# danieleschmidt/spin-torque-rl-gym

Measured on AMD Instinct MI355X. Metric: env_steps_per_sec, higher is better.
Workload: dtype f64

## Files before the change

### spin-torque-rl-gym_amd/csrc/stg_kernels.hpp

```cpp
#pragma once
#include "../../include/spintorque_hip.h"
#include "stg_launch_plan.hpp"
#include "stg_physics.hpp"

#include <hip/hip_runtime.h>

#include <type_traits>

using namespace stg;

struct alignas(16) EnvRec {
    double m[3];
    double tgt[3];
    double etot;
    uint32_t stepw;
    uint32_t rng;
};
static_assert(sizeof(EnvRec) == 64, "state record size");
constexpr uint32_t STG_DONE_BIT = 0x80000000u;

struct StateView {
    EnvRec* rec;
};

// ... 368 lines not shown
            const V3 ref{row[C_REFX], row[C_REFY], row[C_REFZ]};
            const double r = resistance(m, (int)row[C_DEVTYPE], row[C_RP], row[C_RAP], row[C_TMR], ref, row[C_RSERIES]);
            const double v = J * r * row[C_AREA];
            energy = (v * v) / r * T;
        }
        if (so.ok) {
            const double inv = rsqrt_fast(dot(so.m, so.m));
            m = V3{so.m.x * inv, so.m.y * inv, so.m.z * inv};
        }
        etot += energy;
        step += 1;
        rng += 1;
        const double align = dot(m, tgt);
        is_success = align >= a.c.thr;
        reward = 10.0 * (is_success ? 10.0 : 0.0);
        reward += (-a.c.w_energy) * (-energy / 1e-12);
        reward += (align - prev_align);
        if (isnan(reward) || isinf(reward)) reward = -1.0;
        reward = fmin(fmax(reward, -1e6), 1e6);
        truncated = step >= a.c.max_steps;
        st = so.ok ? (so.resets > 0 ? STG_STATUS_RESET : STG_STATUS_OK) : STG_STATUS_NOOP;
        c_steps += 1; c_sub += (unsigned long long)so.work; c_noop += so.ok ? 0 : 1;
        done = is_success || truncated;
    }
    const bool do_reset = a.autoreset && done && live;
    if (wr && do_reset && a.final_obs) {
        if (a.records) {
            float o[12];
            make_obs(o, m, tgt, row, a.c, step, etot, J, T);
            float2* fo = (float2*)(a.final_obs + (ko * N + i) * 12);
#pragma unroll
            for (int q = 0; q < 6; ++q) fo[q] = make_float2(o[2 * q], o[2 * q + 1]);
        } else {
            write_obs(a.final_obs + ko * 12 * N, N, i, m, tgt, row, a.c, step, etot, J, T);
        }
    }
    if (do_reset) {
        device_reset_draw(a.c.seed, env_id, rng, a.c, true, true, m, tgt);
        etot = 0.0; step = 0; done = false;
        J = 0.0; T = 0.0;
    }
    if (wr) {
        if (a.records) {
            write_record((char*)a.obs + ko * N * STG_RECORD_BYTES, i, m, tgt, row, a.c, step, etot, J, T, (float)reward,
                         (is_success ? 1u : 0u) | (truncated ? 0x100u : 0u) | ((uint32_t)st << 16));
        } else {
            write_obs(a.obs + ko * 12 * N, N, i, m, tgt, row, a.c, step, etot, J, T);
            a.reward[ko * N + i] = (float)reward;
            a.term[ko * N + i] = is_success ? 1 : 0;
            a.trunc[ko * N + i] = truncated ? 1 : 0;
        }
        if (a.reward64) a.reward64[ko * N + i] = reward;
        if (a.energy) a.energy[ko * N + i] = energy;
        if (a.status) a.status[ko * N + i] = st;
    }
}

constexpr int REFILL_STRIPES = 64;
constexpr int REFILL_CURSOR_STRIDE = 16;

template <bool THERMAL, bool MULTI, bool AXIS_Z, typename AT, bool IDS>
__device__ __forceinline__ void refill_wave(const StepArgs& a, int64_t w, int64_t nw, int64_t blk0, int64_t nblk_q, int lane, const double* s_tab,
                                            unsigned long long& c_steps, unsigned long long& c_sub, unsigned long long& c_noop) {
    const int64_t N = a.N;
    const int64_t tiles = (N + TILE_ENVS - 1) / TILE_ENVS;
    if (w == 0 && lane < REFILL_STRIPES) a.refill_cursor_next[lane * REFILL_CURSOR_STRIDE] = 0ull;
    const AT* act = (const AT*)a.actions;
    const Recorder norec{};
    const LlgsEnergyK noek{};
    const Dp5Tab tb = make_dp5_tab();
    InlineNormals ns;

    int64_t i = 0, o = 0;
    bool has_env = false;
    double J = 0.0, T = 0.0;
    V3 e_tgt{0.0, 0.0, 1.0};
    double e_etot = 0.0;
    int32_t e_step = 0;
    uint32_t e_rng = 0;
    bool e_skip = false;
    const double* row = a.ctab;
    LlgsK k = load_llgs(row);
    LlgsLane L;
    L.active = false; L.idle = true; L.rejected = false; L.attempts = 0; L.npts = 0;
    L.y = L.f = L.m0 = V3{0.0, 0.0, 1.0};
    L.t = L.T = L.h_abs = L.min_step = L.bJ = L.bpJ = 0.0;
    V3 out_m{0.0, 0.0, 1.0};

    auto take = [&](int64_t p, bool want) {
        const int64_t idx = blk0 + (p >> 6);
        const bool valid_blk = want && (p >> 6) < nblk_q;
        const int64_t slot = (valid_blk ? refill_slot_base(idx, tiles) : 0) + (p & 63);
        const bool valid = valid_blk && slot < N;
        if (!valid) return;
        if constexpr (IDS) {
            o = a.perm ? (int64_t)a.perm[slot] : slot;
            const uint32_t id = a.ids[o];
            if ((int64_t)id >= a.n_state) { write_bad_id(a, o); return; }
            i = (int64_t)id;
        } else {
            i = a.perm ? (int64_t)a.perm[slot] : slot;
        }
        V3 m;
        bool done;
        load_state(a.s, i, m, e_tgt, e_etot, e_step, e_rng, done);
        const uint32_t rng = e_rng;
        if (a.perm) {
            typedef typename std::conditional<std::is_same<AT, double>::value, double2, float2>::type AT2;
            const AT2 aa = ((const AT2*)a.act_sorted)[slot];
            parse_action<AT>(aa.x, aa.y, a.c.max_current, a.c.max_duration, J, T);
        } else {
            const int64_t p = IDS ? o : i;
            parse_action<AT>(act[p], act[N + p], a.c.max_current, a.c.max_duration, J, T);
        }
        if (MULTI) {
            const int c = (int)a.cls[i];
            row = s_tab + (c < a.ncls ? c : 0) * C_COUNT;
            k = load_llgs(row);
        }
        const RngKey rk{a.c.seed, (uint64_t)(a.env_id0 + i), rng};
        e_skip = a.c.skip_done && done;
        llgs_lane_begin<THERMAL, false, AXIS_Z>(L, out_m, m, J, T, k, row[C_BETA], row[C_BETAP], a.c.rtol, a.c.atol, a.c.max_step, rk,
                                                norec, noek, ns, !e_skip);
        has_env = true;
    };
    auto finish = [&]() {
        const SolveOut so = llgs_lane_finish<false>(L, out_m, norec, noek, ns);
        V3 m = L.m0, tgt = e_tgt;
        double etot = e_etot;
        int32_t step = e_step;
        uint32_t rng = e_rng;
        bool done = e_skip;
        env_step_tail(a, IDS ? o : i, 0, true, true, !e_skip, row, (uint64_t)(a.env_id0 + i), m, tgt, etot, step, rng, done, J, T, so, c_steps, c_sub, c_noop);
        store_state(a.s, i, m, tgt, etot, step, rng, done);
        has_env = false;
        L.active = false;
    };

    take(w * 64 + lane, true);
    const int64_t n_rest = nblk_q > nw ? nblk_q - nw : 0;
    static_assert(REFILL_STRIPES == 64, "one lane per stripe when a wavefront looks for a stripe that still has entries");
    int stripe = (int)(w % REFILL_STRIPES);
    bool queue_open = true;
    int64_t loc_q = 0, loc_end = 0;
    int loc_stripe = 0, full_streak = 0;
    bool more = n_rest > 0;
    const int check = a.refill_check > 0 ? a.refill_check : 1;
    for (;;) {
        LlgsMasks M = llgs_masks_open(L);
        for (int c = 0; c < check; ++c) {
            llgs_lane_gate<false>(L, M, (int32_t)a.c.max_attempts);
            if (M.active == 0ull) break;
            V3 z2{0.0, 0.0, 0.0}, z3{0.0, 0.0, 0.0};
            llgs_lane_attempt<THERMAL, false, AXIS_Z, false>(L, M, 0, out_m, k, tb, a.c.rtol, a.c.atol, a.c.max_step, norec, noek, ns, z2, z3);
        }
        llgs_masks_close(L, M);
        const bool fin = has_env && !L.active;
        if (__ballot(fin) != 0ull || (more && __ballot(!has_env) != 0ull)) {
            if (fin) finish();
            const unsigned long long takers = __ballot(!has_env);
            if (more && takers != 0ull) {
                const int n_take = (int)__builtin_popcountll(takers), first = (int)__builtin_ctzll(takers);
                const int rank = (int)__builtin_popcountll(takers & ((1ull << lane) - 1ull));
                const int64_t avail = loc_end - loc_q;
                const int need_new = n_take > avail ? (int)(n_take - avail) : 0;
                int64_t new_q = 0;
                const int new_stripe = stripe;
                if (need_new > 0 && queue_open) {
                    const int reserve = (takers == ~0ull && full_streak >= 1) ? 4 * 64 : need_new;
                    unsigned long long base = 0;
                    if (lane == first) base = atomicAdd(a.refill_cursor + stripe * REFILL_CURSOR_STRIDE, (unsigned long long)reserve);
                    base = (unsigned long long)__shfl((long long)base, first);
                    new_q = (int64_t)base;
                    const int64_t stripe_end = ((n_rest - stripe + REFILL_STRIPES - 1) / REFILL_STRIPES) * 64;
                    int64_t new_end = new_q + reserve;
                    if (new_end >= stripe_end) {
                        new_end = stripe_end;
                        const int64_t end_l = ((n_rest - lane + REFILL_STRIPES - 1) / REFILL_STRIPES) * 64;
                        const unsigned long long cur_l = __hip_atomic_load(a.refill_cursor + lane * REFILL_CURSOR_STRIDE, __ATOMIC_RELAXED, __HIP_MEMORY_SCOPE_AGENT);
                        unsigned long long open_s = __ballot((int64_t)cur_l < end_l);
                        open_s &= ~(1ull << stripe);
                        if (open_s == 0ull) queue_open = false;
                        else {
                            const unsigned long long after = stripe == 63 ? 0ull : (open_s >> (stripe + 1)) << (stripe + 1);
                            stripe = (int)__builtin_ctzll(after != 0ull ? after : open_s);
                        }
                    }
                    const bool from_old = rank < avail;
                    const int64_t q = from_old ? loc_q + rank : new_q + (rank - avail);
                    const int st = from_old ? loc_stripe : new_stripe;
                    const int64_t r = (q >> 6) * REFILL_STRIPES + st;
                    take((nw + r) * 64 + (q & 63), !has_env && r < n_rest && (from_old || q < new_end));
                    loc_q = new_q + need_new < new_end ? new_q + need_new : new_end;
                    loc_end = new_end;
                    loc_stripe = new_stripe;
                } else {
                    const int64_t q = loc_q + rank;
                    const int64_t r = (q >> 6) * REFILL_STRIPES + loc_stripe;
                    take((nw + r) * 64 + (q & 63), !has_env && q < loc_end && r < n_rest);
                    loc_q = loc_q + n_take < loc_end ? loc_q + n_take : loc_end;
                }
                more = queue_open || loc_q < loc_end;
                full_streak = takers == ~0ull ? full_streak + 1 : 0;
            }
        }
        if (__ballot(has_env) == 0ull && !more) break;
    }
}

template <int SOLVER, bool THERMAL, int MULTI, bool AXIS_Z, bool DEVPHYS, typename AT, bool PC, int WGW, bool IDS>
#ifndef STG_STEP_ATTR
#define STG_STEP_ATTR
#endif
__global__ void __launch_bounds__(PC ? 2 * WGW * 64 : WGW * 64, (SOLVER != STG_SOLVER_RK45 && !THERMAL && !DEVPHYS && AXIS_Z && MULTI != 2 && !(MULTI && WGW == 1)) ? 4 : 1) STG_STEP_ATTR
stg_step_kernel(const StepArgs a) {
#pragma clang fp contract(off)
    static_assert(!PC || THERMAL, "wave specialisation only exists for the thermal kernels");
    extern __shared__ double s_tab[];
    constexpr bool FIELD = SOLVER == STG_SOLVER_RK45;
    using NT = typename std::conditional<FIELD, double, float>::type;
    constexpr bool BARRIER = SOLVER != STG_SOLVER_RK4;
    constexpr int DEPTH = BARRIER ? 2 : 4;
    constexpr int RING = DEPTH * (FIELD ? SHARED_CHUNK_RK45 : SHARED_CHUNK_FIXED) * 64;
    static_assert(!PC || WGW == 1, "the wave-specialised form is one integrating + one producing wavefront");
    __shared__ NT s_norm[PC ? RING : 1];
    __shared__ int s_hs[2], s_go[2 * WGW];
    __shared__ unsigned long long s_cnt[(PC ? 2 : 1) * WGW * 3];
    __shared__ uint32_t s_rng[PC ? WGW * 64 : 1];
    const int lane = (int)(threadIdx.x & 63u);
    const int wave = __builtin_amdgcn_readfirstlane((int)(threadIdx.x >> 6));
    bool paired = PC;
    int64_t hyb_slot = 0;
    if (PC && a.hybrid) hyb_slot = stg_hybrid_block(blockIdx.x, wave, (uint32_t)(a.hybrid - 1), (a.N + TILE_ENVS - 1) / TILE_ENVS, paired);
    const bool producer = PC && paired && wave >= WGW;
    const int cw = producer ? (2 * WGW - 1 - wave) : (wave < WGW ? wave : wave - WGW);
    record_placement(a.placement, wave, lane, producer);
    const int64_t lane_slot = ((PC && a.hybrid) ? hyb_slot
                                                : stg_slot_block<WGW>(blockIdx.x, (uint32_t)((a.N + WGW * 64 - 1) / (WGW * 64)), a.perm != nullptr, cw, PC,
                                                                      (uint32_t)a.snake_rounds) * 64) + lane;
    const bool in_list = lane_slot < a.N;
    const int64_t o = in_list ? (a.perm ? (int64_t)a.perm[lane_slot] : lane_slot) : 0;
    const uint32_t id = (IDS && in_list) ? a.ids[o] : 0u;
    const bool bad = IDS && in_list && (int64_t)id >= a.n_state;
    if (bad && !producer) write_bad_id(a, o);
    const bool live = in_list && !bad;
    const int64_t i = IDS ? (live ? (int64_t)id : 0) : o;
    constexpr int ENV_LAYOUT = SOLVER == STG_SOLVER_RK45 ? ENV_LAYOUT_LLGS : (DEVPHYS ? ENV_LAYOUT_DEV : ENV_LAYOUT_CORE);
    double own_row[MULTI == 2 ? C_COUNT : 1];
    const double* row;
    if constexpr (MULTI == 2) {
        stg_device_params p;
        load_env_params<ENV_LAYOUT>(a.ep, i, p);
        derive_row(p, a.ep.gamma, a.ep.temperature, own_row);
        row = own_row;
    } else {
        row = class_row<MULTI != 0>(a.ctab, a.cls, a.ncls, i, live, s_tab, a.ep, ENV_LAYOUT);
    }
    if (!PC && !live) return;
    if (PC && !paired && !live) return;
    const int64_t N = a.N;
    const uint64_t env_id = (uint64_t)(a.env_id0 + i);

    if (producer) {
        constexpr int n_first = SOLVER == STG_SOLVER_RK45 ? 6 : SHARED_CHUNK_FIXED;
        static_assert(3 * SHARED_SUBS3 == SHARED_CHUNK_FIXED, "chunk size of the 3-normal sub-steps");
        constexpr int n_chunk = SOLVER == STG_SOLVER_RK45 ? SHARED_CHUNK_RK45 : n_first;
        const double ghs = FIELD ? load_llgs(row).ghs : 0.0;
        for (int k = 0; k < a.K; ++k) {
            __syncthreads();
            const int p = (k & 1) * WGW;
            if (!any_flag<WGW>(lds_flag(s_go + p))) continue;
            const RngKey rk{a.c.seed, env_id, s_rng[cw * 64 + lane]};
            produce_normals<NT, FIELD, DEPTH, BARRIER>(s_norm, s_hs, lane, rk, n_first, n_chunk, ghs);
        }
        record_retired(a.placement, wave, lane, 0ull);
        return;
    }

    V3 m, tgt;
    double etot;
    int32_t step;
    uint32_t rng;
    bool done;
    load_state(a.s, i, m, tgt, etot, step, rng, done);
    const AT* act = (const AT*)a.actions;
    const Recorder norec{};
    unsigned long long c_steps = 0, c_sub = 0, c_noop = 0;

    for (int k = 0; k < a.K; ++k) {
        double J, T;
        if (k == 0 && a.perm) {
            typedef typename std::conditional<std::is_same<AT, double>::value, double2, float2>::type AT2;
            const AT2 aa = ((const AT2*)a.act_sorted)[live ? lane_slot : 0];
            parse_action<AT>(aa.x, aa.y, a.c.max_current, a.c.max_duration, J, T);
        } else {
            parse_action<AT>(act[((int64_t)k * 2 + 0) * N + o], act[((int64_t)k * 2 + 1) * N + o], a.c.max_current,
                             a.c.max_duration, J, T);
        }
        const bool last = (k == a.K - 1);
        const int64_t ko = a.out_every ? k : 0;
        const bool wr = (a.out_every || last) && live;
        const bool lane_solves = live && !(a.c.skip_done && done);
        const RngKey rk{a.c.seed, env_id, rng};
        SolveOut so{m, 0, 0, 0, false};
        if (PC && paired) {
            SharedNormalsT<NT, FIELD, DEPTH, BARRIER> shared{s_norm, s_hs, lane, 0, 0, 1};
            const int p = (k & 1) * WGW;
// ... 130 lines not shown
```

### spin-torque-rl-gym_amd/csrc/stg_physics.hpp

```cpp
#pragma once

#include <hip/hip_runtime.h>
#include <stdint.h>
#include <type_traits>

#include "stg_minstep.hpp"

namespace stg {

enum ClassConst : int {
    C_EX = 0, C_EY, C_EZ,
    C_HK,
    C_MS,
    C_ALPHA,
    C_GEFF,
    C_POL,
    C_MSV,
    C_HS_SIMPLE,
    C_RX, C_RY, C_RZ,
    C_DX, C_DY, C_DZ,
    C_HEX,
    C_BETA, C_BETAP,
    C_GAMMA,
    C_HS_LLGS,
    C_KUV,
    C_EDEMAG,
    C_NX, C_NY, C_NZ,
    C_AREA, C_RP, C_RAP, C_TMR,
    C_REFX, C_REFY, C_REFZ,
    C_RSERIES,
    C_DEVTYPE,
    C_VALID,
    C_SOT_DL, C_SOT_FL,
    C_SIGX, C_SIGY, C_SIGZ,
    C_KU,
    C_VCMA_XI, C_VCMA_TD2,
    C_VCMA_VBD,
    C_MU0MS,
    C_COUNT
};

template <class P>
__host__ __device__ inline void derive_row(const P& p, double gamma, double temperature, double* r) {
#pragma clang fp contract(off)
    const double mu0 = 4 * 3.14159265358979323846 * 1e-7;
    const double en = sqrt((p.easy_axis[0] * p.easy_axis[0] + p.easy_axis[1] * p.easy_axis[1]) + p.easy_axis[2] * p.easy_axis[2]);
    r[C_EX] = p.easy_axis[0] / en; r[C_EY] = p.easy_axis[1] / en; r[C_EZ] = p.easy_axis[2] / en;
    r[C_HK] = (2 * p.ku) / (mu0 * p.ms);
    r[C_MS] = p.ms;
    r[C_ALPHA] = p.damping;
    r[C_GEFF] = gamma / (1 + p.damping * p.damping);
    r[C_POL] = p.polarization;
    r[C_MSV] = p.ms * p.volume;
    r[C_HS_SIMPLE] = sqrt(2 * p.damping * 1.38e-23 * temperature / (mu0 * p.ms * p.volume * gamma));
    r[C_RX] = p.easy_axis[0]; r[C_RY] = p.easy_axis[1]; r[C_RZ] = p.easy_axis[2];
    r[C_DX] = -p.ms * p.demag[0]; r[C_DY] = -p.ms * p.demag[1]; r[C_DZ] = -p.ms * p.demag[2];
    r[C_HEX] = p.a_ex > 0 ? (2 * p.a_ex / (mu0 * p.ms)) * 0.1 : 0.0;
    r[C_BETA] = p.polarization * gamma / (2 * p.ms * p.volume);
    r[C_BETAP] = 0.1 * r[C_BETA];
    r[C_GAMMA] = gamma;
    r[C_HS_LLGS] = sqrt(2 * p.damping * 1.380649e-23 * temperature / (gamma * mu0 * p.ms * p.volume));
    r[C_KUV] = p.ku * p.volume;
    r[C_EDEMAG] = 0.5 * mu0 * (p.ms * p.ms) * p.volume;
    r[C_NX] = p.demag[0]; r[C_NY] = p.demag[1]; r[C_NZ] = p.demag[2];
    r[C_AREA] = p.area; r[C_RP] = p.r_p; r[C_RAP] = p.r_ap;
    r[C_TMR] = (p.r_ap - p.r_p) / p.r_p;
    const double rn = sqrt((p.ref_m[0] * p.ref_m[0] + p.ref_m[1] * p.ref_m[1]) + p.ref_m[2] * p.ref_m[2]);
    r[C_REFX] = p.ref_m[0] / rn; r[C_REFY] = p.ref_m[1] / rn; r[C_REFZ] = p.ref_m[2] / rn;
    r[C_RSERIES] = p.r_series;
    r[C_DEVTYPE] = (double)p.dev_type;
    r[C_VALID] = p.params_valid ? 1.0 : 0.0;
    r[C_SOT_DL] = p.sot_tau_dl; r[C_SOT_FL] = p.sot_tau_fl;
    r[C_SIGX] = p.sot_sigma[0]; r[C_SIGY] = p.sot_sigma[1]; r[C_SIGZ] = p.sot_sigma[2];
    r[C_KU] = p.ku;
    r[C_VCMA_XI] = p.vcma_xi;
    r[C_VCMA_TD2] = p.vcma_td * p.vcma_td;
    r[C_VCMA_VBD] = p.vcma_vbd;
    r[C_MU0MS] = mu0 * p.ms;
}

struct V3 {
    double x, y, z;
};

__device__ __forceinline__ double mul_x(double a, double b) {
#pragma clang fp contract(off)
    const double r = a * b;
    return r;
}
__device__ __forceinline__ double add_x(double a, double b) {
#pragma clang fp contract(off)
    const double r = a + b;
    return r;
}
__device__ __forceinline__ double sub_x(double a, double b) {
#pragma clang fp contract(off)
    const double r = a - b;
    return r;
}

__device__ __forceinline__ double rsqrt_fast(double s) {
    const double y = __builtin_amdgcn_rsq(s);
    const double e = __builtin_fma(-(s * y), y, 1.0);
    return __builtin_fma(y * e, __builtin_fma(0.375, e, 0.5), y);
}

__device__ __forceinline__ double vgpr_const(double c) {
    asm volatile("" : "+v"(c));
    return c;
}

__device__ __forceinline__ double fmax_abs(double a, double b) {
    double r;
    asm("v_max_f64 %0, |%1|, |%2|" : "=v"(r) : "v"(a), "v"(b));
    return r;
}

__device__ __forceinline__ void commit_step(unsigned long long mask, double& d0, double s0, double& d1, double s1, double& d2, double s2,
                                            double& d3, double s3, double& d4, double s4, double& d5, double s5, double& d6, double s6,
                                            double& min_step, double& h, double unit) {
    unsigned long long saved;
    int e;
    asm("s_and_saveexec_b64 %[sv], %[m]\n\t"
        "v_mov_b64 %[d0], %[s0]\n\t"
        "v_mov_b64 %[d1], %[s1]\n\t"
        "v_mov_b64 %[d2], %[s2]\n\t"
        "v_mov_b64 %[d3], %[s3]\n\t"
        "v_mov_b64 %[d4], %[s4]\n\t"
        "v_mov_b64 %[d5], %[s5]\n\t"
        "v_mov_b64 %[d6], %[s6]\n\t"
        "v_frexp_exp_i32_f64 %[e], %[s0]\n\t"
        "v_max_i32 %[e], %[fl], %[e]\n\t"
        "v_ldexp_f64 %[ms], %[u], %[e]\n\t"
        "v_max_f64 %[h], %[h], %[ms]\n\t"
        "s_mov_b64 exec, %[sv]"
        : [d0] "+v"(d0), [d1] "+v"(d1), [d2] "+v"(d2), [d3] "+v"(d3), [d4] "+v"(d4), [d5] "+v"(d5), [d6] "+v"(d6), [ms] "+v"(min_step),
          [h] "+v"(h), [e] "=&v"(e), [sv] "=&s"(saved)
        : [s0] "v"(s0), [s1] "v"(s1), [s2] "v"(s2), [s3] "v"(s3), [s4] "v"(s4), [s5] "v"(s5), [s6] "v"(s6), [u] "v"(unit), [m] "s"(mask),
          [fl] "n"(MIN_STEP_EXP_FLOOR)
        : "scc");
}

__device__ __forceinline__ double rcp_fast(double x) {
    const double y = __builtin_amdgcn_rcp(x);
    return __builtin_fma(y, __builtin_fma(-x, y, 1.0), y);
}

__device__ __forceinline__ double inv_tenth_root(double e2) {
    const double y = (double)__builtin_amdgcn_exp2f(-0.1f * __builtin_amdgcn_logf((float)e2));
    const double y2 = y * y, y4 = y2 * y2, y8 = y4 * y4;
    const double e = __builtin_fma(-e2, y8 * y2, 1.0);
    return __builtin_fma(y * e, __builtin_fma(0.055, e, 0.1), y);
}

__device__ __forceinline__ double fifth_root(double x) {
    int e;
    const double mant = frexp(x, &e);
    const double t = -0.2 * ((double)e + (double)__builtin_amdgcn_logf((float)mant));
    const double ti = rint(t);
    double r = ldexp((double)__builtin_amdgcn_exp2f((float)(t - ti)), (int)ti);
    const double r2 = r * r, r4 = r2 * r2;
    const double err = __builtin_fma(-x, r4 * r, 1.0);
    r = __builtin_fma(r * err, __builtin_fma(0.12, err, 0.2), r);
    const double q2 = r * r;
    return x * (q2 * q2);
}

__device__ __forceinline__ V3 cross(const V3& a, const V3& b) {
#pragma clang fp contract(off)
    return V3{__builtin_fma(a.y, b.z, -(a.z * b.y)), __builtin_fma(a.z, b.x, -(a.x * b.z)), __builtin_fma(a.x, b.y, -(a.y * b.x))};
}
__device__ __forceinline__ double dot(const V3& a, const V3& b) {
#pragma clang fp contract(off)
    return __builtin_fma(a.z, b.z, __builtin_fma(a.y, b.y, a.x * b.x));
}
__device__ __forceinline__ V3 scale3(double c, const V3& z) {
#pragma clang fp contract(off)
    return V3{c * z.x, c * z.y, c * z.z};
}
__device__ __forceinline__ bool finite3(const V3& a) { return isfinite(a.x) && isfinite(a.y) && isfinite(a.z); }

__device__ __forceinline__ void philox4x32_10(uint32_t c0, uint32_t c1, uint32_t c2, uint32_t c3, uint32_t k0,
                                              uint32_t k1, uint32_t (&out)[4]) {
#pragma unroll
    for (int r = 0; r < 10; ++r) {
        const uint32_t hi0 = __umulhi(0xD2511F53u, c0), lo0 = 0xD2511F53u * c0;
        const uint32_t hi1 = __umulhi(0xCD9E8D57u, c2), lo1 = 0xCD9E8D57u * c2;
        const uint32_t n0 = hi1 ^ c1 ^ k0, n2 = hi0 ^ c3 ^ k1;
        c0 = n0; c1 = lo1; c2 = n2; c3 = lo0;
        k0 += 0x9E3779B9u; k1 += 0xBB67AE85u;
    }
    out[0] = c0; out[1] = c1; out[2] = c2; out[3] = c3;
}

struct NormalStream {
    uint32_t s0, s1, s2, s3;
    float carry;
    __device__ __forceinline__ void init(uint64_t seed, uint64_t env_id, uint32_t env_step, uint32_t tag) {
        uint32_t r[4];
        philox4x32_10((uint32_t)env_id, (uint32_t)(env_id >> 32), env_step, tag, (uint32_t)seed, (uint32_t)(seed >> 32), r);
        s0 = r[0]; s1 = r[1]; s2 = r[2]; s3 = r[3] | 1u;
        carry = 0.0f;
    }
    __device__ __forceinline__ uint32_t next() {
        const uint32_t result = s0 + s3;
        const uint32_t t = s1 << 9;
        s2 ^= s0; s3 ^= s1; s1 ^= s2; s0 ^= s3; s2 ^= t;
        s3 = (s3 << 11) | (s3 >> 21);
        return result;
    }
    __device__ __forceinline__ float uniform() {
        return __uint_as_float(__builtin_amdgcn_alignbit(0x7fu, next(), 9u)) - 0.99999994f;
    }
    typedef float f32x2 __attribute__((ext_vector_type(2)));
    __device__ __forceinline__ void pair(float& a, float& b) {
        float t, c, s_;
        pair_head(t, c, s_);
        finish_pair(t, c, s_, a, b);
    }
    __device__ __forceinline__ void pair_head(float& t, float& c, float& s_) {
        f32x2 u{__uint_as_float(__builtin_amdgcn_alignbit(0x7fu, next(), 9u)), __uint_as_float(__builtin_amdgcn_alignbit(0x7fu, next(), 9u))};
        u = u - f32x2{0.99999994f, 0.99999994f};
        t = -1.3862943611198906f * __builtin_amdgcn_logf(u.x);
        c = __builtin_amdgcn_cosf(u.y);
        s_ = __builtin_amdgcn_sinf(u.y);
    }
    static __device__ __forceinline__ void finish_pair(float t, float c, float s_, float& a, float& b) {
        const float r = __builtin_amdgcn_sqrtf(t);
        const f32x2 cs = f32x2{c, s_} * f32x2{r, r};
        a = cs.x;
        b = cs.y;
    }
    __device__ __forceinline__ V3 draw3_even() {
        float a, b, c, d;
        pair(a, b);
        pair(c, d);
        carry = d;
        return V3{(double)a, (double)b, (double)c};
    }
    __device__ __forceinline__ V3 draw3_odd() {
        float a, b;
        pair(a, b);
        return V3{(double)carry, (double)a, (double)b};
    }
};

struct RngKey {
    uint64_t seed, env_id;
    uint32_t env_step;
};

struct InlineNormals {
    static constexpr bool kShared = false, kScaled = false;
    NormalStream ns;
    __device__ __forceinline__ void begin(const RngKey& rk) { ns.init(rk.seed, rk.env_id, rk.env_step, 0u); }
    __device__ __forceinline__ V3 draw(bool even) { return even ? ns.draw3_even() : ns.draw3_odd(); }
    static constexpr bool broken = false;
    __device__ __forceinline__ void peek() {}
    __device__ __forceinline__ bool chunk_end(bool lane_continues) { return lane_continues; }
    __device__ __forceinline__ bool chunk_end_wave(bool mine) { return mine; }
};

constexpr int SHARED_SUBS_RK4 = 2;
constexpr int SHARED_SUBS3 = 4 * SHARED_SUBS_RK4;
constexpr int SHARED_CHUNK_FIXED = 12 * SHARED_SUBS_RK4;
constexpr int SHARED_CHUNK_RK45 = 18;
constexpr int PC_STOP = 1 << 30;
constexpr int PC_SPIN_CAP = 1 << 22;

typedef __attribute__((address_space(3))) int lds_int;
__device__ __forceinline__ volatile lds_int* lds_flag(const int* p) { return (volatile lds_int*)p; }

template <int WGW>
__device__ __forceinline__ bool any_flag(volatile lds_int* f) {
    int v = f[0];
#pragma unroll
    for (int j = 1; j < WGW; ++j) v |= f[j];
    return v != 0;
}
__device__ __forceinline__ int pc_load(const int* p) {
    return __builtin_amdgcn_readfirstlane(__hip_atomic_load(p, __ATOMIC_ACQUIRE, __HIP_MEMORY_SCOPE_WORKGROUP));
}
__device__ __forceinline__ void pc_store(int* p, int v) {
    __hip_atomic_store(p, v, __ATOMIC_RELEASE, __HIP_MEMORY_SCOPE_WORKGROUP);
}

template <typename T, bool SCALED, int DEPTH, bool BARRIER>
struct SharedNormalsT {
    static constexpr int CHUNK = SCALED ? SHARED_CHUNK_RK45 : SHARED_CHUNK_FIXED;
    static_assert(!BARRIER || DEPTH == 2, "the barrier form runs the producer exactly one chunk ahead");
    static constexpr bool kShared = true, kScaled = SCALED;
    const T* buf;
    int* hs;
    int lane, it, idx, seen;
    bool broken;
    static constexpr bool kToggle = BARRIER && SCALED;
    int slot_el, flag_el;
    __device__ __forceinline__ void begin(const RngKey&) {
        it = 0; idx = 0; seen = 1; broken = false;
        if (kToggle) {
            static_assert(((CHUNK * 64) & 63) == 0, "the slot bit and the lane bits are disjoint");
            slot_el = lane; flag_el = 0;
            asm volatile("" : "+v"(slot_el), "+v"(flag_el));
        }
    }
    __device__ __forceinline__ V3 draw(bool) {
        const T* b = kToggle ? buf + slot_el + idx * 64 : buf + ((it & (DEPTH - 1)) * CHUNK + idx) * 64 + lane;
        idx += 3;
        return V3{(double)b[0], (double)b[64], (double)b[128]};
    }
    __device__ __forceinline__ void peek() {
        if (!BARRIER) seen = __hip_atomic_load(hs, __ATOMIC_RELAXED, __HIP_MEMORY_SCOPE_WORKGROUP);
    }
    __device__ __forceinline__ bool chunk_end(bool lane_continues) { return chunk_end_wave(__ballot(lane_continues) != 0ull); }
    __device__ __forceinline__ bool chunk_end_wave(bool mine) {
        if (BARRIER) {
            lds_flag(hs)[kToggle ? flag_el : (it & 1)] = mine ? 1 : 0;
            if (kToggle) { flag_el ^= 1; slot_el ^= CHUNK * 64; }
            __syncthreads();
            ++it;
            idx = 0;
            return mine;
        }
        ++it;
        idx = 0;
        pc_store(hs + 1, it | (mine ? 0 : PC_STOP));
        int have = __builtin_amdgcn_readfirstlane(seen);
        if (__builtin_expect(mine && have <= it, 0)) {
            int spins = 0;
#pragma unroll 1
            do {
                if (spins) __builtin_amdgcn_s_sleep(1);
                have = pc_load(hs);
            } while (have <= it && ++spins <= PC_SPIN_CAP);
            broken = broken || have <= it;
        }
        seen = have;
        __builtin_amdgcn_fence(__ATOMIC_ACQUIRE, "workgroup");
        return mine && !broken;
    }
};

template <typename T, bool SCALED, int DEPTH, bool BARRIER>
__device__ __forceinline__ void produce_normals(T* buf, int* hs, int lane, const RngKey& rk, int n_first, int n_chunk, double c) {
    NormalStream ns;
    ns.init(rk.seed, rk.env_id, rk.env_step, 0u);
    bool even = true;
    auto fill = [&](int slot, int count) {
        T* b = buf + (slot * (SCALED ? SHARED_CHUNK_RK45 : SHARED_CHUNK_FIXED)) * 64 + lane;
        for (int j = 0; j < count; j += 3) {
            V3 z = even ? ns.draw3_even() : ns.draw3_odd();
            if (SCALED) z = scale3(c, z);
            even = !even;
            b[(j + 0) * 64] = (T)z.x; b[(j + 1) * 64] = (T)z.y; b[(j + 2) * 64] = (T)z.z;
        }
    };
    fill(0, n_first);
    if (!BARRIER) pc_store(hs, 1);
    __syncthreads();
    if (BARRIER) {
        for (int k = 1;; ++k) {
            fill(k & 1, n_chunk);
            __syncthreads();
            if (lds_flag(hs)[(k - 1) & 1] == 0) return;
        }
    }
    for (int k = 1;; ++k) {
        int v = pc_load(hs + 1);
#pragma unroll 1
        for (int spins = 0; (v & (PC_STOP - 1)) < k - DEPTH + 1 && !(v & PC_STOP); ++spins) {
            if (spins > PC_SPIN_CAP) return;
            __builtin_amdgcn_s_sleep(1);
            v = pc_load(hs + 1);
        }
        if (v & PC_STOP) return;
        fill(k & (DEPTH - 1), n_chunk);
        pc_store(hs, k + 1);
    }
}

struct SimpleK {
    V3 e;
    double ghk;
    double gdm;
    double alpha;
    double ghs;
};
__device__ __forceinline__ SimpleK make_simple(const V3& e, double hk, double ms, double alpha, double geff, double hs) {
#pragma clang fp contract(off)
    return SimpleK{e, -geff * hk, geff * ms, alpha, -geff * hs};
}
struct LlgsK {
    V3 r;
    V3 gd;
    double ghk, ghex;
    double alpha;
    double ghs;
    double gz;
    double agz;
};
__device__ __forceinline__ LlgsK make_llgs(const V3& r, const V3& d, double hk, double hex, double alpha, double gamma, double hs) {
#pragma clang fp contract(off)
    const double ng = -gamma;
    const double gz = ng * ((hk * r.z) * r.z + d.z);
    return LlgsK{r, V3{ng * d.x, ng * d.y, ng * d.z}, ng * hk, ng * hex, alpha, ng * hs, gz, alpha * gz};
}


template <bool THERMAL, bool AXIS_Z>
__device__ __forceinline__ V3 simple_rhs(const V3& m, const SimpleK& k, double ghk, double aJ, const V3& z) {
#pragma clang fp contract(off)
    if (AXIS_Z) {
        const double gz = (ghk + k.gdm) * m.z;
        V3 p;
        if (THERMAL) {
            const V3 g{k.ghs * z.x, k.ghs * z.y, __builtin_fma(k.ghs, z.z, gz)};
            p = cross(m, g);
        } else {
            p = V3{m.y * gz, -(m.x * gz), 0.0};
        }
        const double wx = __builtin_fma(k.alpha, p.x, aJ * m.y), wy = __builtin_fma(k.alpha, p.y, -(aJ * m.x));
        if (THERMAL) {
            const double wz = k.alpha * p.z;
            return V3{__builtin_fma(m.y, wz, __builtin_fma(-m.z, wy, p.x)), __builtin_fma(m.z, wx, __builtin_fma(-m.x, wz, p.y)),
                      __builtin_fma(m.x, wy, __builtin_fma(-m.y, wx, p.z))};
        }
        return V3{__builtin_fma(-m.z, wy, p.x), __builtin_fma(m.z, wx, p.y), __builtin_fma(m.x, wy, -(m.y * wx))};
    }
    const V3 t = cross(m, k.e);
    const double c = ghk * dot(m, k.e);
    const double d = k.gdm * m.z;
    V3 p;
    if (THERMAL) {
        const V3 g{__builtin_fma(k.ghs, z.x, c * k.e.x), __builtin_fma(k.ghs, z.y, c * k.e.y),
                   __builtin_fma(k.ghs, z.z, __builtin_fma(c, k.e.z, d))};
        p = cross(m, g);
    } else {
        p = V3{__builtin_fma(c, t.x, d * m.y), __builtin_fma(c, t.y, -(d * m.x)), c * t.z};
    }
    const V3 w{__builtin_fma(k.alpha, p.x, aJ * t.x), __builtin_fma(k.alpha, p.y, aJ * t.y),
               __builtin_fma(k.alpha, p.z, aJ * t.z)};
    return V3{__builtin_fma(m.y, w.z, __builtin_fma(-m.z, w.y, p.x)), __builtin_fma(m.z, w.x, __builtin_fma(-m.x, w.z, p.y)),
              __builtin_fma(m.x, w.y, __builtin_fma(-m.y, w.x, p.z))};
}

struct DevTorque {
    double sdl, sfl;
    V3 sigma;
    double ghk_pulse;
    bool any_sot;
};

__device__ __forceinline__ double vcma_keff(double volt, double ku, double xi, double td2, double vbd) {
    const double v = volt < -vbd ? -vbd : (volt > vbd ? vbd : volt);
    const double keff = ku + (-xi * fabs(v) / td2);
    return fmax(keff, -0.5 * ku);
}

template <bool THERMAL, bool AXIS_Z, bool DEVPHYS>
__device__ __forceinline__ V3 simple_stage(const V3& m, const SimpleK& k, double aJ, const V3& z, const DevTorque& dv,
                                           bool on) {
#pragma clang fp contract(off)
    if (!DEVPHYS) return simple_rhs<THERMAL, AXIS_Z>(m, k, k.ghk, aJ, z);
    V3 f = simple_rhs<THERMAL, AXIS_Z>(m, k, on ? dv.ghk_pulse : k.ghk, aJ, z);
    if (dv.any_sot) {
        const double a = on ? dv.sdl : 0.0, b = on ? dv.sfl : 0.0;
        const V3 sxm = cross(dv.sigma, m);
        f = V3{f.x + __builtin_fma(a, sxm.x, b * dv.sigma.x), f.y + __builtin_fma(a, sxm.y, b * dv.sigma.y),
               f.z + __builtin_fma(a, sxm.z, b * dv.sigma.z)};
    }
    return f;
// ... 166 lines not shown
    const double inv = rsqrt_fast(ss);
    V3 m{y.x * inv, y.y * inv, y.z * inv};
    if (CHECKED) {
        const bool unit = ss > 1e-24;
        if (__builtin_expect(__ballot(!unit) != 0ull, 0)) m = V3{unit ? m.x : 0.0, unit ? m.y : 0.0, unit ? m.z : 1.0};
    }
    if (AXIS_Z) {
        const double u = __builtin_fma(k.gz, m.z, bpJ);
        const double w = __builtin_fma(k.agz, m.z, bJ);
        if (!THERMAL) {
            const double c = m.z * w;
            return V3{__builtin_fma(m.x, c, m.y * u), __builtin_fma(m.y, c, -(m.x * u)), __builtin_fma(m.z, c, -w)};
        }
        const double uz = ht.z + u;
        const V3 W{k.alpha * ht.x, k.alpha * ht.y, __builtin_fma(k.alpha, ht.z, w)};
        const double s = dot(m, W);
        return V3{__builtin_fma(m.x, s, __builtin_fma(m.y, uz, __builtin_fma(-m.z, ht.y, -W.x))),
                  __builtin_fma(m.y, s, __builtin_fma(m.z, ht.x, __builtin_fma(-m.x, uz, -W.y))),
                  __builtin_fma(m.z, s, __builtin_fma(m.x, ht.y, __builtin_fma(-m.y, ht.x, -W.z)))};
    }
    const double c = k.ghk * dot(m, k.r);
    V3 g{(c * k.r.x + k.gd.x * m.x) + k.ghex * m.x, (c * k.r.y + k.gd.y * m.y) + k.ghex * m.y,
         (c * k.r.z + k.gd.z * m.z) + k.ghex * m.z};
    if (THERMAL) g = V3{g.x + ht.x, g.y + ht.y, g.z + ht.z};
    const V3 U{g.x, g.y, g.z + bpJ};
    const V3 W{k.alpha * g.x, k.alpha * g.y, __builtin_fma(k.alpha, g.z, bJ)};
    const double s = dot(m, W);
    return V3{__builtin_fma(m.x, s, __builtin_fma(m.y, U.z, __builtin_fma(-m.z, U.y, -W.x))),
              __builtin_fma(m.y, s, __builtin_fma(m.z, U.x, __builtin_fma(-m.x, U.z, -W.y))),
              __builtin_fma(m.z, s, __builtin_fma(m.x, U.y, __builtin_fma(-m.y, U.x, -W.z)))};
}

struct LlgsEnergyK {
    double kuv, edemag;
    V3 r, nfac;
};
__device__ __forceinline__ double llgs_energy(const V3& m, const LlgsEnergyK& k) {
    const double ct = dot(m, k.r);
    return -k.kuv * (ct * ct) + k.edemag * (k.nfac.x * (m.x * m.x) + k.nfac.y * (m.y * m.y) + k.nfac.z * (m.z * m.z));
}

__device__ __forceinline__ double llgs_torque_norms(const V3& m, double bJ, double bpJ) {
#pragma clang fp contract(off)
    const V3 mxp{m.y, -m.x, 0.0};
    const V3 mm = cross(m, mxp);
    const V3 a{bJ * mm.x, bJ * mm.y, bJ * mm.z}, b{bpJ * mxp.x, bpJ * mxp.y, bpJ * mxp.z};
    return sqrt((a.x * a.x + a.y * a.y) + a.z * a.z) + sqrt((b.x * b.x + b.y * b.y) + b.z * b.z);
}

__device__ __forceinline__ double rms3(const V3& a) { return sqrt(dot(a, a)) / 1.7320508075688772; }

struct Dp5Tab {
    double A51, A52, A53, A54, A61, A62, A63, A64, A65, E1, E3, E4, E5, E6, E7;
    double ms_unit;
};
__device__ __forceinline__ Dp5Tab make_dp5_tab() {
    Dp5Tab t;
    t.A51 = vgpr_const(19372.0 / 6561); t.A52 = vgpr_const(-25360.0 / 2187); t.A53 = vgpr_const(64448.0 / 6561); t.A54 = vgpr_const(-212.0 / 729);
    t.A61 = vgpr_const(9017.0 / 3168); t.A62 = vgpr_const(-355.0 / 33); t.A63 = vgpr_const(46732.0 / 5247); t.A64 = vgpr_const(49.0 / 176);
    t.A65 = vgpr_const(-5103.0 / 18656);
    t.E1 = vgpr_const(-71.0 / 57600); t.E3 = vgpr_const(71.0 / 16695); t.E4 = vgpr_const(-71.0 / 1920); t.E5 = vgpr_const(17253.0 / 339200);
    t.E6 = vgpr_const(-22.0 / 525); t.E7 = vgpr_const(1.0 / 40);
    t.ms_unit = vgpr_const(MIN_STEP_UNIT);
    return t;
}

struct LlgsLane {
    V3 y, f;
    V3 m0;
    double t, T, h_abs, min_step;
    double bJ, bpJ;
    int32_t attempts;
    int32_t npts;
    bool idle;
    bool rejected, active;
};

typedef unsigned long long lanemask;
struct LlgsMasks {
    lanemask active, pacc;
};
__device__ __forceinline__ bool lane_in(lanemask m) { return __builtin_amdgcn_inverse_ballot_w64(m); }
__device__ __forceinline__ LlgsMasks llgs_masks_open(const LlgsLane& L) { return LlgsMasks{__ballot(L.active), __ballot(!L.rejected)}; }
__device__ __forceinline__ void llgs_masks_close(LlgsLane& L, const LlgsMasks& M) {
    L.active = lane_in(M.active);
    L.rejected = !lane_in(M.pacc);
}

template <bool RECORD>
__device__ __forceinline__ void llgs_lane_emit(LlgsLane& L, V3& out_m, const Recorder& rec, const LlgsEnergyK& ek) {
    const double inv = rsqrt_fast(dot(L.y, L.y));
    out_m = V3{L.y.x * inv, L.y.y * inv, L.y.z * inv};
    if (RECORD) rec.put(L.npts, L.t, out_m, rec.e ? llgs_energy(out_m, ek) : 0.0, rec.tq ? llgs_torque_norms(out_m, L.bJ, L.bpJ) : 0.0);
    ++L.npts;
}

template <bool THERMAL, bool AXIS_Z, bool CHECKED = true>
__device__ __forceinline__ V3 llgs_fun(const LlgsLane& L, const LlgsK& k, const V3& y, const V3& ht, bool on) {
    return llgs_rhs<THERMAL, AXIS_Z, CHECKED>(y, k, on ? L.bJ : 0.0, on ? L.bpJ : 0.0, ht);
}
template <bool THERMAL, class NSRC>
__device__ __forceinline__ V3 llgs_draw(NSRC& ns, const LlgsK& k, bool even) {
    if (!THERMAL) return V3{0.0, 0.0, 0.0};
    return NSRC::kScaled ? ns.draw(even) : scale3(k.ghs, ns.draw(even));
}

template <bool THERMAL, bool RECORD, bool AXIS_Z, class NSRC>
__device__ __forceinline__ void llgs_lane_begin(LlgsLane& L, V3& out_m, const V3& m0, double J, double T, const LlgsK& k, double beta,
                                                double betap, double rtol, double atol, double max_step, const RngKey& rk,
                                                const Recorder& rec, const LlgsEnergyK& ek, NSRC& ns, bool enabled) {
    const bool useJ = !(fabs(J) < 1e-12);
    L.bJ = useJ ? beta * J : 0.0;
    L.bpJ = useJ ? betap * J : 0.0;
    L.m0 = m0;
    L.T = T;
    if (THERMAL) ns.begin(rk);
    const double n0 = rsqrt_fast(dot(m0, m0));
    L.y = V3{m0.x * n0, m0.y * n0, m0.z * n0};
    L.t = 0.0;
    L.npts = 0;
    if (RECORD) llgs_lane_emit<RECORD>(L, out_m, rec, ek); else ++L.npts;
    L.f = llgs_fun<THERMAL, AXIS_Z>(L, k, L.y, llgs_draw<THERMAL>(ns, k, true), true);
    double h_abs;
    {
        const V3& y = L.y;
        const V3& f = L.f;
        const V3 sc{atol + fabs(y.x) * rtol, atol + fabs(y.y) * rtol, atol + fabs(y.z) * rtol};
        const V3 isc{rcp_fast(sc.x), rcp_fast(sc.y), rcp_fast(sc.z)};
        const double d0 = rms3(V3{y.x * isc.x, y.y * isc.y, y.z * isc.z});
        const double d1 = rms3(V3{f.x * isc.x, f.y * isc.y, f.z * isc.z});
        double h0 = (d0 < 1e-5 || d1 < 1e-5) ? 1e-6 : (0.01 * d0) * rcp_fast(d1);
        h0 = fmin(h0, T);
        const V3 y1{y.x + h0 * f.x, y.y + h0 * f.y, y.z + h0 * f.z};
        const V3 f1 = llgs_fun<THERMAL, AXIS_Z>(L, k, y1, llgs_draw<THERMAL>(ns, k, false), true);
        const double d2 = rms3(V3{(f1.x - f.x) * isc.x, (f1.y - f.y) * isc.y, (f1.z - f.z) * isc.z}) * rcp_fast(h0);
        const double h1 = (d1 <= 1e-15 && d2 <= 1e-15) ? fmax(1e-6, h0 * 1e-3) : fifth_root(0.01 * rcp_fast(fmax(d1, d2)));
        h_abs = fmin(fmin(100.0 * h0, h1), fmin(T, max_step));
    }
    L.rejected = false;
    L.attempts = 0;
    L.min_step = min_step_at(L.t);
    L.h_abs = h_abs > max_step ? max_step : (h_abs < L.min_step ? L.min_step : h_abs);
    L.active = enabled && (L.t != T);
    L.idle = !L.active;
}

template <bool UNIFORM_IT>
__device__ __forceinline__ void llgs_lane_gate(const LlgsLane& L, LlgsMasks& M, int32_t max_attempts) {
    lanemask stop = __ballot(L.h_abs < L.min_step);
    if (!UNIFORM_IT) stop |= __ballot(L.attempts >= max_attempts);
    M.active &= ~stop;
}

template <bool THERMAL, bool RECORD, bool AXIS_Z, bool UNIFORM_IT, class NSRC>
__device__ __forceinline__ void llgs_lane_attempt(LlgsLane& L, LlgsMasks& M, int32_t it, V3& out_m, const LlgsK& k, const Dp5Tab& tb, double rtol,
                                                  double atol, double max_step, const Recorder& rec, const LlgsEnergyK& ek, NSRC& ns, V3 z2, V3 z3) {
    constexpr double A21 = 1.0 / 5;
    constexpr double A31 = 3.0 / 40, A32 = 9.0 / 40;
    constexpr double A41 = 44.0 / 45, A42 = -56.0 / 15, A43 = 32.0 / 9;
    constexpr double B1 = 35.0 / 384, B3 = 500.0 / 1113, B4 = 125.0 / 192, B5 = -2187.0 / 6784, B6 = 11.0 / 84;
    const double A51 = tb.A51, A52 = tb.A52, A53 = tb.A53, A54 = tb.A54, A61 = tb.A61, A62 = tb.A62, A63 = tb.A63, A64 = tb.A64, A65 = tb.A65;
    const double E1 = tb.E1, E3 = tb.E3, E4 = tb.E4, E5 = tb.E5, E6 = tb.E6, E7 = tb.E7;
    const double T = L.T;
    const bool active = lane_in(M.active);
    const V3 y = L.y;
    const double t = L.t;
    auto fun = [&](const V3& yy, const V3& ht, bool on) -> V3 { return llgs_fun<THERMAL, AXIS_Z, false>(L, k, yy, ht, on); };
    auto draw = [&](bool even) -> V3 { return llgs_draw<THERMAL>(ns, k, even); };
    if (UNIFORM_IT) L.attempts = active ? it + 1 : L.attempts; else L.attempts += active ? 1 : 0;
    const double t_new = fmin(add_x(t, L.h_abs), T);
    const double h = sub_x(t_new, t);
    const double h_try = fabs(h);
    const bool on_end = add_x(t, h) <= T;
    const V3 k1 = L.f;
    if (THERMAL && !NSRC::kShared) { z2 = draw(true); z3 = draw(false); }
    const V3 k2 = fun(V3{y.x + (k1.x * A21) * h, y.y + (k1.y * A21) * h, y.z + (k1.z * A21) * h}, z2, true);
    const V3 z4 = draw(true);
    const V3 k3 = fun(V3{y.x + (k1.x * A31 + k2.x * A32) * h, y.y + (k1.y * A31 + k2.y * A32) * h,
                         y.z + (k1.z * A31 + k2.z * A32) * h}, z3, true);
    const V3 z5 = draw(false);
    const V3 k4 = fun(V3{y.x + (k1.x * A41 + k2.x * A42 + k3.x * A43) * h, y.y + (k1.y * A41 + k2.y * A42 + k3.y * A43) * h,
                         y.z + (k1.z * A41 + k2.z * A42 + k3.z * A43) * h}, z4, true);
    const V3 z6 = draw(true);
    const V3 k5 = fun(V3{y.x + (k1.x * A51 + k2.x * A52 + k3.x * A53 + k4.x * A54) * h,
                         y.y + (k1.y * A51 + k2.y * A52 + k3.y * A53 + k4.y * A54) * h,
                         y.z + (k1.z * A51 + k2.z * A52 + k3.z * A53 + k4.z * A54) * h}, z5, true);
    if (THERMAL) ns.peek();
    const V3 z7 = draw(false);
    const V3 k6 = fun(V3{y.x + (k1.x * A61 + k2.x * A62 + k3.x * A63 + k4.x * A64 + k5.x * A65) * h,
                         y.y + (k1.y * A61 + k2.y * A62 + k3.y * A63 + k4.y * A64 + k5.y * A65) * h,
                         y.z + (k1.z * A61 + k2.z * A62 + k3.z * A63 + k4.z * A64 + k5.z * A65) * h}, z6, on_end);
    const V3 y_new{y.x + h * (k1.x * B1 + k3.x * B3 + k4.x * B4 + k5.x * B5 + k6.x * B6),
                   y.y + h * (k1.y * B1 + k3.y * B3 + k4.y * B4 + k5.y * B5 + k6.y * B6),
                   y.z + h * (k1.z * B1 + k3.z * B3 + k4.z * B4 + k5.z * B5 + k6.z * B6)};
    const V3 f_new = fun(y_new, z7, on_end);
    const V3 ev{(k1.x * E1 + k3.x * E3 + k4.x * E4 + k5.x * E5 + k6.x * E6 + f_new.x * E7) * h,
                (k1.y * E1 + k3.y * E3 + k4.y * E4 + k5.y * E5 + k6.y * E6 + f_new.y * E7) * h,
                (k1.z * E1 + k3.z * E3 + k4.z * E4 + k5.z * E5 + k6.z * E6 + f_new.z * E7) * h};
    const V3 sc{atol + fmax_abs(y.x, y_new.x) * rtol, atol + fmax_abs(y.y, y_new.y) * rtol, atol + fmax_abs(y.z, y_new.z) * rtol};
    const V3 q{ev.x * rcp_fast(sc.x), ev.y * rcp_fast(sc.y), ev.z * rcp_fast(sc.z)};
    const double err2 = dot(q, q) * (1.0 / 3.0);
    const double err = err2;
    const lanemask accm = M.active & __ballot(err < 1.0);
    const bool acc = lane_in(accm);
    const double r9 = 0.9 * inv_tenth_root(err);
    const double fa = fmin(lane_in(M.pacc) ? 10.0 : 1.0, r9);
    const double fr = fmax(0.2, r9);
    double h_next = fmin(h_try * (acc ? fa : fr), max_step);
    commit_step(accm, L.t, t_new, L.y.x, y_new.x, L.y.y, y_new.y, L.y.z, y_new.z, L.f.x, f_new.x, L.f.y, f_new.y, L.f.z, f_new.z,
                L.min_step, h_next, tb.ms_unit);
    L.h_abs = h_next;
    if (RECORD) { if (acc) llgs_lane_emit<RECORD>(L, out_m, rec, ek); } else L.npts += acc ? 1 : 0;
    M.pacc = accm;
    M.active &= __ballot(L.t != T);
}

template <bool RECORD, class NSRC>
__device__ __forceinline__ SolveOut llgs_lane_finish(LlgsLane& L, V3& out_m, const Recorder& rec, const LlgsEnergyK& ek, const NSRC& ns) {
    SolveOut o{L.m0, 0, 0, 0, false};
    if (!RECORD) { llgs_lane_emit<RECORD>(L, out_m, rec, ek); --L.npts; }
    o.m = out_m;
    o.n = L.npts - 1;
    o.work = L.attempts;
    const bool ok = L.idle || L.t == L.T;
    o.ok = ok && !ns.broken;
    if (!ok) o.m = L.m0;
    return o;
}

template <bool THERMAL, bool RECORD, bool AXIS_Z, class NSRC>
__device__ __forceinline__ SolveOut llgs_solve(const V3& m0, double J, double T, const LlgsK& k, double beta,
                                               double betap, double rtol, double atol, double max_step,
                                               int64_t max_attempts, const RngKey& rk, const Recorder& rec,
                                               const LlgsEnergyK& ek, NSRC& ns, bool enabled) {
    const Dp5Tab tb = make_dp5_tab();
    const V3 zero{0.0, 0.0, 0.0};
    LlgsLane L;
    V3 out_m = m0;
    llgs_lane_begin<THERMAL, RECORD, AXIS_Z>(L, out_m, m0, J, T, k, beta, betap, rtol, atol, max_step, rk, rec, ek, ns, enabled);
    LlgsMasks M = llgs_masks_open(L);
    atol = vgpr_const(atol);
    const int32_t budget = (int32_t)max_attempts;
    int32_t it = 0;
    bool wave_go = true;
    if (NSRC::kShared) wave_go = ns.chunk_end_wave(M.active != 0ull);
    if (wave_go)
    for (;;) {
      V3 z2 = zero, z3 = zero;
      if (THERMAL && NSRC::kShared) { z2 = llgs_draw<THERMAL>(ns, k, true); z3 = llgs_draw<THERMAL>(ns, k, false); }
      llgs_lane_gate<true>(L, M, budget);
      if (!NSRC::kShared && M.active == 0ull) break;
      llgs_lane_attempt<THERMAL, RECORD, AXIS_Z, true>(L, M, it, out_m, k, tb, rtol, atol, max_step, rec, ek, ns, z2, z3);
      ++it;
      const bool go = it < budget;
      if (NSRC::kShared) { if (!ns.chunk_end_wave(go && M.active != 0ull)) break; }
      else if (!go) break;
    }
    llgs_masks_close(L, M);
    return llgs_lane_finish<RECORD>(L, out_m, rec, ek, ns);
}

__device__ __forceinline__ double resistance(const V3& m_in, int dev_type, double r_p, double r_ap, double tmr,
                                             const V3& ref, double r_series) {
#pragma clang fp contract(off)
    if (dev_type == 0) {
        const double inv = rsqrt_fast(dot(m_in, m_in));
        const V3 m{m_in.x * inv, m_in.y * inv, m_in.z * inv};
        const double r = r_p * (1.0 + tmr * (1.0 - dot(m, ref)) * 0.5);
        return fmax(r, r_p * 0.5);
    }
    double r = r_p + (r_ap - r_p) * (1.0 - dot(m_in, ref)) * 0.5;
    if (dev_type == 1) r = r + r_series;
    return fmax(r, 1.0);
}

template <typename AT>
__device__ __forceinline__ void parse_action(AT a0, AT a1, double max_current, double max_duration, double& J, double& T) {
    const AT cmax = (AT)1e8, dmin = (AT)1e-12, dmax = (AT)1e-6;
    if (!isnan(a0)) a0 = a0 < -cmax ? -cmax : (a0 > cmax ? cmax : a0);
    if (!isnan(a1)) a1 = a1 < dmin ? dmin : (a1 > dmax ? dmax : a1);
    if (isnan(a0) || isnan(a1) || isinf(a0) || isinf(a1)) { a0 = (AT)0; a1 = dmin; }
    const double j = (double)a0, t = (double)a1;
    J = j < -max_current ? -max_current : (j > max_current ? max_current : j);
    T = t < 1e-12 ? 1e-12 : (t > max_duration ? max_duration : t);
}

__device__ __forceinline__ float obs_cast(double v) {
    const float f = (float)v;
    return isnan(f) ? 0.0f : (isinf(f) ? (f > 0 ? 1e6f : -1e6f) : f);
}

}
```

Baseline: 43.14 million.

## Split chunk barrier into post/meet and overlap step-size math with it

The shared-noise chunk barrier is split into a post phase (write the LDS flag) and a meet phase (syncthreads plus flag read). The adaptive step-size controller's tenth-root computation is split into log, residual and Newton stages that are interleaved around the barrier, and the next noise draws are issued inside the meet callback. This is meant to hide barrier and transcendental latency behind independent work, at the cost of more live registers and more complex control flow. The h clamp is now applied after the controller instead of inside the commit asm.

```diff
diff --git a/spin-torque-rl-gym_amd/csrc/stg_kernels.hpp b/spin-torque-rl-gym_amd/csrc/stg_kernels.hpp
--- a/spin-torque-rl-gym_amd/csrc/stg_kernels.hpp
+++ b/spin-torque-rl-gym_amd/csrc/stg_kernels.hpp
@@ -544,7 +544,7 @@
             llgs_lane_gate<false>(L, M, (int32_t)a.c.max_attempts);
             if (M.active == 0ull) break;
             V3 z2{0.0, 0.0, 0.0}, z3{0.0, 0.0, 0.0};
-            llgs_lane_attempt<THERMAL, false, AXIS_Z, false>(L, M, 0, out_m, k, tb, a.c.rtol, a.c.atol, a.c.max_step, norec, noek, ns, z2, z3);
+            llgs_lane_attempt<THERMAL, false, AXIS_Z, false>(L, M, 0, out_m, k, tb, a.c.rtol, a.c.atol, a.c.max_step, norec, noek, ns, z2, z3, [] {}, [] {});
         }
         llgs_masks_close(L, M);
         const bool fin = has_env && !L.active;
diff --git a/spin-torque-rl-gym_amd/csrc/stg_physics.hpp b/spin-torque-rl-gym_amd/csrc/stg_physics.hpp
--- a/spin-torque-rl-gym_amd/csrc/stg_physics.hpp
+++ b/spin-torque-rl-gym_amd/csrc/stg_physics.hpp
@@ -116,40 +116,48 @@
     return r;
 }
 
-__device__ __forceinline__ void commit_step(unsigned long long mask, double& d0, double s0, double& d1, double s1, double& d2, double s2,
-                                            double& d3, double s3, double& d4, double s4, double& d5, double s5, double& d6, double s6,
-                                            double& min_step, double& h, double unit) {
+__device__ __forceinline__ void commit_state(unsigned long long mask, double& d0, double s0, double& d1, double s1, double& d2, double s2,
+                                             double& d3, double s3, double& d4, double s4, double& d5, double s5, double& d6, double s6,
+                                             double& min_step, double& clamp, double unit) {
     unsigned long long saved;
     int e;
-    asm("s_and_saveexec_b64 %[sv], %[m]\n\t"
+    asm volatile("s_and_saveexec_b64 %[sv], %[m]\n\t"
         "v_mov_b64 %[d0], %[s0]\n\t"
+        "v_frexp_exp_i32_f64 %[e], %[s0]\n\t"
         "v_mov_b64 %[d1], %[s1]\n\t"
+        "v_max_i32 %[e], %[fl], %[e]\n\t"
         "v_mov_b64 %[d2], %[s2]\n\t"
+        "v_ldexp_f64 %[ms], %[u], %[e]\n\t"
         "v_mov_b64 %[d3], %[s3]\n\t"
+        "v_mov_b64 %[cl], %[ms]\n\t"
         "v_mov_b64 %[d4], %[s4]\n\t"
         "v_mov_b64 %[d5], %[s5]\n\t"
         "v_mov_b64 %[d6], %[s6]\n\t"
-        "v_frexp_exp_i32_f64 %[e], %[s0]\n\t"
-        "v_max_i32 %[e], %[fl], %[e]\n\t"
-        "v_ldexp_f64 %[ms], %[u], %[e]\n\t"
-        "v_max_f64 %[h], %[h], %[ms]\n\t"
         "s_mov_b64 exec, %[sv]"
         : [d0] "+v"(d0), [d1] "+v"(d1), [d2] "+v"(d2), [d3] "+v"(d3), [d4] "+v"(d4), [d5] "+v"(d5), [d6] "+v"(d6), [ms] "+v"(min_step),
-          [h] "+v"(h), [e] "=&v"(e), [sv] "=&s"(saved)
+          [cl] "+v"(clamp), [e] "=&v"(e), [sv] "=&s"(saved)
         : [s0] "v"(s0), [s1] "v"(s1), [s2] "v"(s2), [s3] "v"(s3), [s4] "v"(s4), [s5] "v"(s5), [s6] "v"(s6), [u] "v"(unit), [m] "s"(mask),
           [fl] "n"(MIN_STEP_EXP_FLOOR)
         : "scc");
 }
+__device__ __forceinline__ double clamp_step(double h, double clamp) {
+    double r;
+    asm("v_max_f64 %0, %1, %2" : "=v"(r) : "v"(h), "v"(clamp));
+    return r;
+}
 
 __device__ __forceinline__ double rcp_fast(double x) {
     const double y = __builtin_amdgcn_rcp(x);
     return __builtin_fma(y, __builtin_fma(-x, y, 1.0), y);
 }
 
-__device__ __forceinline__ double inv_tenth_root(double e2) {
-    const double y = (double)__builtin_amdgcn_exp2f(-0.1f * __builtin_amdgcn_logf((float)e2));
+__device__ __forceinline__ float inv_tenth_root_log(double e2) { return __builtin_amdgcn_logf((float)e2); }
+__device__ __forceinline__ double inv_tenth_root_residual(double e2, float lg, double& y) {
+    y = (double)__builtin_amdgcn_exp2f(-0.1f * lg);
     const double y2 = y * y, y4 = y2 * y2, y8 = y4 * y4;
-    const double e = __builtin_fma(-e2, y8 * y2, 1.0);
+    return __builtin_fma(-e2, y8 * y2, 1.0);
+}
+__device__ __forceinline__ double inv_tenth_root_newton(double y, double e) {
     return __builtin_fma(y * e, __builtin_fma(0.055, e, 0.1), y);
 }
 
@@ -259,6 +267,8 @@
     __device__ __forceinline__ void peek() {}
     __device__ __forceinline__ bool chunk_end(bool lane_continues) { return lane_continues; }
     __device__ __forceinline__ bool chunk_end_wave(bool mine) { return mine; }
+    __device__ __forceinline__ void chunk_post(bool) {}
+    __device__ __forceinline__ bool chunk_meet(bool mine) { return mine; }
 };
 
 constexpr int SHARED_SUBS_RK4 = 2;
@@ -314,9 +324,17 @@
     }
     __device__ __forceinline__ bool chunk_end(bool lane_continues) { return chunk_end_wave(__ballot(lane_continues) != 0ull); }
     __device__ __forceinline__ bool chunk_end_wave(bool mine) {
+        chunk_post(mine);
+        return chunk_meet(mine);
+    }
+    __device__ __forceinline__ void chunk_post(bool mine) {
         if (BARRIER) {
             lds_flag(hs)[kToggle ? flag_el : (it & 1)] = mine ? 1 : 0;
             if (kToggle) { flag_el ^= 1; slot_el ^= CHUNK * 64; }
+        }
+    }
+    __device__ __forceinline__ bool chunk_meet(bool mine) {
+        if (BARRIER) {
             __syncthreads();
             ++it;
             idx = 0;
@@ -789,9 +807,10 @@
     M.active &= ~stop;
 }
 
-template <bool THERMAL, bool RECORD, bool AXIS_Z, bool UNIFORM_IT, class NSRC>
+template <bool THERMAL, bool RECORD, bool AXIS_Z, bool UNIFORM_IT, class NSRC, class POST, class MEET>
 __device__ __forceinline__ void llgs_lane_attempt(LlgsLane& L, LlgsMasks& M, int32_t it, V3& out_m, const LlgsK& k, const Dp5Tab& tb, double rtol,
-                                                  double atol, double max_step, const Recorder& rec, const LlgsEnergyK& ek, NSRC& ns, V3 z2, V3 z3) {
+                                                  double atol, double max_step, const Recorder& rec, const LlgsEnergyK& ek, NSRC& ns, V3 z2, V3 z3,
+                                                  POST&& post, MEET&& meet) {
     constexpr double A21 = 1.0 / 5;
     constexpr double A31 = 3.0 / 40, A32 = 9.0 / 40;
     constexpr double A41 = 44.0 / 45, A42 = -56.0 / 15, A43 = 32.0 / 9;
@@ -838,18 +857,28 @@
     const V3 q{ev.x * rcp_fast(sc.x), ev.y * rcp_fast(sc.y), ev.z * rcp_fast(sc.z)};
     const double err2 = dot(q, q) * (1.0 / 3.0);
     const double err = err2;
+    float lg = inv_tenth_root_log(err);
+    asm volatile("" : "+v"(lg));
     const lanemask accm = M.active & __ballot(err < 1.0);
     const bool acc = lane_in(accm);
-    const double r9 = 0.9 * inv_tenth_root(err);
-    const double fa = fmin(lane_in(M.pacc) ? 10.0 : 1.0, r9);
-    const double fr = fmax(0.2, r9);
-    double h_next = fmin(h_try * (acc ? fa : fr), max_step);
-    commit_step(accm, L.t, t_new, L.y.x, y_new.x, L.y.y, y_new.y, L.y.z, y_new.z, L.f.x, f_new.x, L.f.y, f_new.y, L.f.z, f_new.z,
-                L.min_step, h_next, tb.ms_unit);
-    L.h_abs = h_next;
+    const bool prev_acc = lane_in(M.pacc);
+    double clamp = 0.0;
+    commit_state(accm, L.t, t_new, L.y.x, y_new.x, L.y.y, y_new.y, L.y.z, y_new.z, L.f.x, f_new.x, L.f.y, f_new.y, L.f.z, f_new.z,
+                 L.min_step, clamp, tb.ms_unit);
+    asm volatile("" : "+v"(lg));
     if (RECORD) { if (acc) llgs_lane_emit<RECORD>(L, out_m, rec, ek); } else L.npts += acc ? 1 : 0;
     M.pacc = accm;
     M.active &= __ballot(L.t != T);
+    post();
+    double y0;
+    double res = inv_tenth_root_residual(err, lg, y0);
+    asm volatile("" : "+v"(res));
+    meet();
+    const double r9 = 0.9 * inv_tenth_root_newton(y0, res);
+    const double fa = fmin(prev_acc ? 10.0 : 1.0, r9);
+    const double fr = fmax(0.2, r9);
+    const double h_next = fmin(h_try * (acc ? fa : fr), max_step);
+    L.h_abs = clamp_step(h_next, clamp);
 }
 
 template <bool RECORD, class NSRC>
@@ -881,17 +910,27 @@
     int32_t it = 0;
     bool wave_go = true;
     if (NSRC::kShared) wave_go = ns.chunk_end_wave(M.active != 0ull);
-    if (wave_go)
-    for (;;) {
-      V3 z2 = zero, z3 = zero;
+    V3 z2 = zero, z3 = zero;
+    if (wave_go) {
       if (THERMAL && NSRC::kShared) { z2 = llgs_draw<THERMAL>(ns, k, true); z3 = llgs_draw<THERMAL>(ns, k, false); }
-      llgs_lane_gate<true>(L, M, budget);
-      if (!NSRC::kShared && M.active == 0ull) break;
-      llgs_lane_attempt<THERMAL, RECORD, AXIS_Z, true>(L, M, it, out_m, k, tb, rtol, atol, max_step, rec, ek, ns, z2, z3);
-      ++it;
-      const bool go = it < budget;
-      if (NSRC::kShared) { if (!ns.chunk_end_wave(go && M.active != 0ull)) break; }
-      else if (!go) break;
+      V3 z2n = zero, z3n = zero;
+      bool mine = false;
+      auto post = [&]() {
+        ++it;
+        mine = it < budget && (!NSRC::kShared || M.active != 0ull);
+        ns.chunk_post(mine);
+      };
+      auto meet = [&]() {
+        wave_go = ns.chunk_meet(mine);
+        if (THERMAL && NSRC::kShared) { z2n = llgs_draw<THERMAL>(ns, k, true); z3n = llgs_draw<THERMAL>(ns, k, false); }
+      };
+      for (;;) {
+        llgs_lane_gate<true>(L, M, budget);
+        if (!NSRC::kShared && M.active == 0ull) break;
+        llgs_lane_attempt<THERMAL, RECORD, AXIS_Z, true>(L, M, it, out_m, k, tb, rtol, atol, max_step, rec, ek, ns, z2, z3, post, meet);
+        if (!wave_go) break;
+        z2 = z2n; z3 = z3n;
+      }
     }
     llgs_masks_close(L, M);
     return llgs_lane_finish<RECORD>(L, out_m, rec, ek, ns);
```

Result: no change. 43.28 million, median of 6 (+0.3%).
